# MaxLayar/Ray-Tracing-Extended

Hardware: AMD Instinct MI355X
Metric: Mrays/s (higher is better)
Workload: dtype f32; 1 GPU; configs[2]: Chess pieces x17 (100,440 triangles, BVH4), 1920x1080, 64 rays/pixel/frame (1024 spp = 16 frames), 8 bounces, PCG, FLAT_CHUNKS semantics; decomposition=single GPU, rays_per_frame=243378252, triangles=100440, chunks=7448, spheres=0

## Files before the change

ray-tracing-extended_amd/csrc/rt_api.hip:

```cpp
#include <hip/hip_runtime.h>

#include <algorithm>
#include <chrono>
#include <cfloat>
#include <cmath>
#include <condition_variable>
#include <deque>
#include <mutex>
#include <cstdarg>
#include <cstdio>
#include <cstring>
#include <ctime>
#include <string>
#include <thread>
#include <vector>

#include "rt_kernels.hpp"
#include "rt_stream.hpp"
namespace rtk {
const void* stream_kernel(bool counting, bool philox, bool compact, bool triangles);
const void* cam_stream_kernel(bool philox, bool compact, bool triangles);
}
#include "rt_geom.hpp"
#include "rt_bvh_gpu.hpp"
// ... 45 lines not shown
    size_t n_tris = 0, n_chunks = 0, n_spheres = 0;
    float sphere_mag = 0.f;
    bool geom_local = false, xf_dirty = false;
    uint64_t frames_traced = 0, frames_at_world_build = ~0ull;
    std::vector<rt_triangle>       h_local_tris;
    std::vector<rt_local_chunk>    h_lchunks;
    std::vector<rt_mesh_transform> h_xf;
    std::vector<float>             mesh_radius;
    int n_meshes = 0;
    DevBuf<float> d_local_tris;
    DevBuf<uint32_t> d_tri_mesh, d_tri_chunk, d_tri_rank, d_order;
    DevBuf<rtg::MeshXf> d_xf;
    hipEvent_t evg0 = nullptr, evg1 = nullptr;
    hipEvent_t ev_switch = nullptr;

    DevBuf<float4> d_sph_geom, d_sph_mat, d_nodes, d_nodes_h, d_tri_geo, d_tri_nrm, d_chunk_mat, d_chunk_box;
    DevBuf<float>  d_raw_tris;
    DevBuf<uint32_t> d_raw_range;
    DevBuf<float4> d_frame, d_accum;
    DevBuf<uint32_t> d_display;
    DevBuf<float4> d_batch;
    DevBuf<uint32_t> d_tile_order, d_tile_cost, d_tile_hist;
    bool lpt_active = true;
    bool tile_order_valid = false, tile_order_stale = false; int tile_order_n = 0;
    size_t target_pixels = 0;
    int target_w = 0, target_h = 0, target_row0 = 0, target_rows = 0, target_row_stride = 8;
    unsigned int* d_tile_counter = nullptr;
    unsigned long long* d_counters = nullptr;

    rtbvh::Bvh bvh;
    size_t n_nodes = 0;
    rtgb::Workspace bvh_ws;
    float area_at_build = 0.f;
    float area_after_refit = 0.f;
    int opt_device_bvh = -1;
    int opt_bvh_radius = -16;
    int opt_peer_copies = 0;
    int opt_bvh_treelet_ratio = 8, opt_bvh_treelet_isolate = 1, opt_bvh_treelet_first = 1;
    int opt_bvh_treelets = 6;
    int opt_bvh_top = 0;
    int opt_rebuild_percent = 200;
    int n_cu = 0;
    int opt_kernel = -1;
    int auto_choice = -1; double auto_ms[2] = { -1.0, -1.0 };
    unsigned variants_launched = 0;
    int opt_shade_threshold = 48;
    int opt_tile_sync = 1;
    int opt_fetch_guide = 4;
    int opt_fetch_guide_philox = 1;
    int opt_tiles_per_fetch = 16;
    int opt_compact_nodes = 1;
    int opt_stream_tile = 4;
    int opt_node_min = 10;
    int opt_blocks_per_cu = 0;
    int opt_full_sort = 0;
    int opt_tile_lpt = 1;
    int opt_frame_batch = 0;
    int opt_tile_w_log2 = 3;
    int opt_bvh_reinsert = 0;
    int opt_bvh_bins = 32, opt_bvh_cost_exp = 100;
    int opt_max_leaf = 2;
    int opt_bvh_collapse = 0;
    int opt_bvh_node_cost = 130;
    int opt_stream_stack = 0;
    int opt_lds_stack = 0;
    DevBuf<uint32_t> d_gstack;
    DevBuf<uint4> d_primary; DevBuf<float4> d_focus; DevBuf<unsigned int> d_primary_counts;
    std::string primary_key;
    unsigned long long scene_version = 0;
    int opt_primary_lists = 1;
    DevBuf<float> d_park;
    std::vector<rtk::CamRecord> h_cams; DevBuf<rtk::CamRecord> d_cams;
    DevBuf<float4> d_q_rays, d_q_hits; DevBuf<uint8_t> d_q_occ;
    DevBuf<unsigned int> d_q_bound;
    DevBuf<float4> d_aov[RT_AOV_COUNT];
    size_t aov_pixels = 0;
    int aov_w = 0, aov_h = 0, aov_row0 = 0, aov_rows = 0, aov_row_stride = 8;
    rt_aov_info aov{};
    rt_stats stats{};

    std::thread q_thread; bool q_started = false;
    std::mutex q_mu; std::condition_variable q_cv, q_idle;
    struct QItem { int frame; rt_params p; };
    std::deque<QItem> q_frames; bool q_busy = false, q_stop = false;
    rt_params q_tail{};
    int q_rc = 0; std::string q_err;
    int opt_queue_depth = 64;
    int opt_queue_linger_us = 200;
};

namespace {

int fail(rt_ctx* ctx, int code, const char* fmt, ...)
{
    char buf[512];
    va_list ap; va_start(ap, fmt); vsnprintf(buf, sizeof buf, fmt, ap); va_end(ap);
    if (ctx) ctx->err = buf; else g_create_error = buf;
    return code;
}

template <class T> hipError_t upload(rt_ctx* c, DevBuf<T>& d, const std::vector<T>& v)
{
    hipError_t e = d.ensure(v.size());
    if (e == hipSuccess && !v.empty()) e = hipMemcpyAsync(d.p, v.data(), v.size() * sizeof(T), hipMemcpyHostToDevice, c->stream);
    return e;
}
// ... 475 lines not shown
    if (philox && var == Variant::Flat) return fail(c, -2, "the flat validation kernel implements the PCG stream only");
    if (philox) kernel = 1;
    if (philox && (c->target_w > 65535 || c->target_rows > 65535)) return fail(c, -7, "the Philox mode addresses at most 65535 x 65535 pixels per context");
    if (philox && (c->params.numRaysPerPixel > 65000 || c->params.maxBounceCount > 32000))
        return fail(c, -7, "the Philox mode takes at most 65000 rays per pixel per frame and 32000 bounces (sample and bounce share one signed 32-bit register)");
    const bool stream = P.stream = kernel == 1 && var != Variant::Flat && c->params.numRaysPerPixel >= 1
                                   && c->target_w <= 65535 && c->target_rows <= 65535;
    const bool tile_kernel = P.tile_kernel = !stream && var != Variant::Flat;
    F.stack_cap = tile_kernel ? tile_stack_cap(c)
                              : std::max(1, c->bvh.maxStack) + (stream ? 3 : 0);
    const bool six_waves = stream && !philox && var == Variant::Fast && c->opt_compact_nodes != 0 && c->n_nodes > 0;
    const int stream_stack = c->opt_stream_stack > 0 ? c->opt_stream_stack : (six_waves ? 24 : 30);
    const bool stream_spill = stream && F.stack_cap > stream_stack;
    if (stream_spill) F.stack_cap = stream_stack;
    F.full_sort = c->opt_full_sort;
    bool fixed_origin = camera_origin_is_fixed(c->params);
    if (cams) for (int f = 0; f < n_frames; ++f) fixed_origin = fixed_origin && camera_origin_is_fixed(cams[f]);
    F.fixed_origin = fixed_origin ? 1 : 0;
    F.out_frame = c->d_frame.p; F.accum = c->d_accum.p;
    F.tile_counter = c->d_tile_counter; F.counters = c->d_counters;

    const size_t lds = P.lds = var == Variant::Flat ? 0
                                       : (size_t)F.stack_cap * 64 * sizeof(uint32_t) * rtk::kWavesPerBlock
                                         + (stream ? (size_t)rtk::kGroupMax * sizeof(uint2) * rtk::kWavesPerBlock : 0);
    if (lds > 160 * 1024) return fail(c, -7, "BVH needs a %d-entry traversal stack: exceeds the 160 KiB LDS", F.stack_cap);
    const bool counting = var == Variant::Counting;
    const bool compact = c->opt_compact_nodes != 0;
    P.cam_table = cams != nullptr;
    const void* fn = P.fn = var == Variant::Flat ? (const void*)rtk::k_trace<false, true>
                   : stream ? (cams ? rtk::cam_stream_kernel(philox, compact, c->n_nodes > 0)
                                    : rtk::stream_kernel(counting, philox, compact, c->n_nodes > 0))
                   : c->n_nodes == 0
                            ? dispatch3(counting, false, false, [](auto C, auto, auto) { return (const void*)rtk::k_trace<decltype(C)::value, false, false, 6>; })
                            : dispatch3(counting, false, compact, [](auto C, auto, auto H) { return (const void*)rtk::k_trace<decltype(C)::value, false, decltype(H)::value>; });
    if (lds > 64 * 1024) RT_HIP(c, hipFuncSetAttribute(fn, hipFuncAttributeMaxDynamicSharedMemorySize, (int)lds));
    int per_cu = 0;
    RT_HIP(c, hipOccupancyMaxActiveBlocksPerMultiprocessor(&per_cu, fn, rtk::kBlock, lds));
    if (per_cu < 1) return fail(c, -7, "kernel does not fit a CU (LDS %zu B)", lds);
    P.ntiles = F.tiles_x * F.tiles_y;
    P.sample_lanes_log2 = !philox ? 0 : c->params.numRaysPerPixel >= 16 ? 4 : c->params.numRaysPerPixel >= 4 ? 2 : 0;
    const bool stream_sync = P.stream_sync = stream && (c->opt_tile_sync || philox);
    if (cams && !stream_sync) return fail(c, -7, "per-frame cameras: no k_cam_stream launch for this target");
    const size_t frames_in_queue = ((stream_sync && c->opt_frame_batch != 1) ? (size_t)std::max(1, std::min(n_frames, 64)) : 1) << P.sample_lanes_log2;
    const int want = (int)std::min<size_t>(((size_t)P.ntiles * frames_in_queue + rtk::kWavesPerBlock - 1) / rtk::kWavesPerBlock, (size_t)1 << 20);
    if (c->opt_blocks_per_cu > 0) per_cu = std::min(per_cu, c->opt_blocks_per_cu);
    const int grid = P.grid = std::max(1, std::min(want, per_cu * c->n_cu));
    A.shade_threshold = std::max(1, std::min(64, c->opt_shade_threshold));
    A.total_pixels = (unsigned int)P.ntiles * 64u;
    A.tile_sync = stream_sync ? 1 : 0;
    A.sample_lanes_log2 = P.sample_lanes_log2;
    A.tiles_per_fetch = std::max(1, std::min(rtk::kGroupMax, c->opt_tiles_per_fetch));
    A.guide_div = 1;
    A.node_min = std::max(1, std::min(64, c->opt_node_min));
    const unsigned int gstack_stride = (unsigned int)grid * rtk::kBlock;
    if (philox) {
        RT_HIP(c, c->d_park.ensure((size_t)grid * rtk::kWavesPerBlock * (size_t)A.tiles_per_fetch * 192));
        F.park = c->d_park.p;
    }
    if (stream_spill) {
        RT_HIP(c, c->d_gstack.ensure((size_t)(c->bvh.maxStack + 3 - F.stack_cap) * gstack_stride));
        F.gstack = c->d_gstack.p; F.gstack_stride = gstack_stride;
    }
    if (tile_kernel && c->bvh.maxStack > F.stack_cap) {
        RT_HIP(c, c->d_gstack.ensure((size_t)(c->bvh.maxStack - F.stack_cap) * gstack_stride));
        F.gstack = c->d_gstack.p; F.gstack_stride = gstack_stride;
    }
    if ((tile_kernel || stream_sync) && n_frames > 1 && c->opt_frame_batch != 1) {
        const size_t budget = (size_t)4 << 30;
        const size_t per_frame = c->target_pixels * sizeof(float4);
        int batch = (int)std::min<size_t>((size_t)n_frames, std::max<size_t>(1, budget / per_frame));
        if (c->opt_frame_batch > 1) batch = std::min(batch, c->opt_frame_batch);
        P.batch = batch = std::min(batch, 256);
        if (batch > 1) RT_HIP(c, c->d_batch.ensure((size_t)batch * c->target_pixels));
    }
    return 0;
}

int plan_tile_order(rt_ctx* c, LaunchPlan& P)
{
    const int ntiles = P.ntiles;
    const bool lpt = (P.tile_kernel || P.stream_sync) && c->opt_tile_lpt && ntiles > 1;
    c->lpt_active = lpt;
    if (!lpt) return 0;
    if (c->tile_order_n != ntiles) { c->tile_order_valid = false; c->tile_order_n = ntiles; }
    RT_HIP(c, c->d_tile_cost.ensure(ntiles)); RT_HIP(c, c->d_tile_order.ensure(ntiles));
    if (!c->tile_order_valid || c->tile_order_stale) {
        P.record_costs = true;
        RT_HIP(c, hipMemsetAsync(c->d_tile_cost.p, 0, (size_t)ntiles * sizeof(uint32_t), c->stream));
    }
    P.F.tile_order = c->tile_order_valid ? c->d_tile_order.p : nullptr;
    P.F.tile_cost = P.record_costs ? c->d_tile_cost.p : nullptr;
    return 0;
}

int ensure_primary_lists(rt_ctx* c, LaunchPlan& P)
{
    const bool eligible = P.stream && !P.cam_table && c->opt_primary_lists && c->n_nodes > 0 && P.F.fixed_origin && c->target_pixels > 0
                          && c->bvh.maxStack <= 160;
    if (!eligible) return 0;
    std::string key((const char*)&c->params, sizeof c->params);
    const unsigned long long geo[6] = { c->scene_version, (unsigned long long)c->target_row0, (unsigned long long)c->target_rows,
                                        (unsigned long long)c->target_row_stride, (unsigned long long)c->target_w, (unsigned long long)c->target_h };
    key.append((const char*)geo, sizeof geo);
    if (key != c->primary_key) {
        RT_HIP(c, c->d_primary.ensure(c->target_pixels)); RT_HIP(c, c->d_focus.ensure(c->target_pixels)); RT_HIP(c, c->d_primary_counts.ensure(4));
        RT_HIP(c, hipMemsetAsync(c->d_primary_counts.p, 0, 4 * sizeof(unsigned int), c->stream));
// ... 615 lines not shown
    if (c->geom_local && n_meshes != c->n_meshes) return fail(c, -2, "%d transforms for %d meshes", n_meshes, c->n_meshes);
    c->h_xf.assign(xf, xf + n_meshes);
    c->xf_dirty = true;
    return 0;
}

int rt_read_world_geometry(rt_ctx* c, rt_triangle* tris_out, int n_tris, rt_meshinfo* mi_out, int n_chunks)
{
    if (!c) return -1;
    RT_SETTLE(c);
    if (!c->geom_local) return fail(c, -2, "no local meshes uploaded");
    if (!c->have_params) return fail(c, -2, "rt_set_params has not been called");
    if (n_tris != (int)c->h_local_tris.size() || n_chunks != (int)c->h_lchunks.size()) return fail(c, -2, "size mismatch");
    RT_HIP(c, hipSetDevice(c->device));
    { int r = prepare_scene(c); if (r) return r; }
    if (n_tris) RT_HIP(c, hipMemcpy(tris_out, c->d_raw_tris.p, (size_t)n_tris * sizeof(rt_triangle), hipMemcpyDeviceToHost));
    std::vector<float4> box(2 * (size_t)n_chunks);
    if (n_chunks) RT_HIP(c, hipMemcpy(box.data(), c->d_chunk_box.p, box.size() * sizeof(float4), hipMemcpyDeviceToHost));
    for (int m = 0; m < n_chunks; ++m) {
        const rt_local_chunk& ch = c->h_lchunks[m];
        rt_meshinfo& mi = mi_out[m];
        mi.firstTriangleIndex = ch.firstTriangleIndex; mi.numTriangles = ch.numTriangles; mi.material = ch.material;
        mi.boundsMin[0] = box[2 * m].x; mi.boundsMin[1] = box[2 * m].y; mi.boundsMin[2] = box[2 * m].z;
        mi.boundsMax[0] = box[2 * m + 1].x; mi.boundsMax[1] = box[2 * m + 1].y; mi.boundsMax[2] = box[2 * m + 1].z;
    }
    return 0;
}

int rt_set_option(rt_ctx* c, const char* name, int value)
{
    if (!c) return -1;
    RT_SETTLE(c);
    if (!name) return fail(c, -2, "null option name");
    if (!std::strcmp(name, "kernel")) {
        if (value < -1 || value > 1) return fail(c, -2, "kernel must be -1 (auto), 0 (k_trace) or 1 (k_stream)");
        c->opt_kernel = value;
    }
    else if (!std::strcmp(name, "shade_threshold")) { if (value < 1 || value > 64) return fail(c, -2, "shade_threshold must be in [1,64]"); c->opt_shade_threshold = value; }
    else if (!std::strcmp(name, "stream_stack")) { if (value != 0 && (value < 4 || value > 128)) return fail(c, -2, "stream_stack must be 0 (automatic) or in [4,128]"); c->opt_stream_stack = value; }
    else if (!std::strcmp(name, "lds_stack")) { if (value < 0 || value > 64) return fail(c, -2, "lds_stack must be in [0,64]"); c->opt_lds_stack = value; }
    else if (!std::strcmp(name, "bvh_bins")) { if (value < 2 || value > 128) return fail(c, -2, "bvh_bins must be in [2,128]"); if (value != c->opt_bvh_bins) c->scene_dirty = true; c->opt_bvh_bins = value; }
    else if (!std::strcmp(name, "bvh_reinsert")) { if (value < 0 || value > 16) return fail(c, -2, "bvh_reinsert must be in [0,16]"); if (value != c->opt_bvh_reinsert) c->scene_dirty = true; c->opt_bvh_reinsert = value; }
    else if (!std::strcmp(name, "bvh_cost_exp")) { if (value < 10 || value > 300) return fail(c, -2, "bvh_cost_exp must be in [10,300] (percent)"); if (value != c->opt_bvh_cost_exp) c->scene_dirty = true; c->opt_bvh_cost_exp = value; }
    else if (!std::strcmp(name, "max_leaf")) { if (value < 1 || value > rtbvh::kMaxLeaf) return fail(c, -2, "max_leaf must be in [1,4]"); if (value != c->opt_max_leaf) c->scene_dirty = true; c->opt_max_leaf = value; }
    else if (!std::strcmp(name, "bvh_collapse")) { if (value < 0 || value > 2) return fail(c, -2, "bvh_collapse must be 0 (greedy), 1 (cost-driven, leaves formed by the collapse) or 2 (cost-driven over the split search's leaves)"); if (value != c->opt_bvh_collapse) c->scene_dirty = true; c->opt_bvh_collapse = value; }
    else if (!std::strcmp(name, "bvh_node_cost")) { if (value < 1 || value > 10000) return fail(c, -2, "bvh_node_cost must be in [1,10000] (percent of a triangle test)"); if (value != c->opt_bvh_node_cost) c->scene_dirty = true; c->opt_bvh_node_cost = value; }
    else if (!std::strcmp(name, "tile_w_log2")) { if (value < 0 || value > 6) return fail(c, -2, "tile_w_log2 must be in [0,6]"); c->opt_tile_w_log2 = value; }
    else if (!std::strcmp(name, "tile_lpt")) { c->opt_tile_lpt = value ? 1 : 0; c->tile_order_valid = false; }
    else if (!std::strcmp(name, "frame_batch")) { if (value < 0 || value > 1024) return fail(c, -2, "frame_batch must be in [0,1024]"); c->opt_frame_batch = value; }
    else if (!std::strcmp(name, "fetch_guide")) { if (value < 1 || value > 64) return fail(c, -2, "fetch_guide must be in [1,64]"); c->opt_fetch_guide = value; }
    else if (!std::strcmp(name, "fetch_guide_philox")) { if (value < 1 || value > 64) return fail(c, -2, "fetch_guide_philox must be in [1,64]"); c->opt_fetch_guide_philox = value; }
    else if (!std::strcmp(name, "tiles_per_fetch")) { if (value < 1 || value > 64) return fail(c, -2, "tiles_per_fetch must be in [1,64]"); c->opt_tiles_per_fetch = value; }
    else if (!std::strcmp(name, "node_min")) { if (value < 1 || value > 64) return fail(c, -2, "node_min must be in [1,64]"); c->opt_node_min = value; }
    else if (!std::strcmp(name, "tile_sync")) c->opt_tile_sync = value ? 1 : 0;
    else if (!std::strcmp(name, "compact_nodes")) c->opt_compact_nodes = value ? 1 : 0;
    else if (!std::strcmp(name, "device_bvh")) { if (value < -1 || value > 1) return fail(c, -2, "device_bvh must be -1 (automatic), 0 or 1"); if (value != c->opt_device_bvh) c->scene_dirty = true; c->opt_device_bvh = value; }
    else if (!std::strcmp(name, "bvh_radius")) { if (value == 0 || value < -rtgb::kMaxRadius || value > rtgb::kMaxRadius) return fail(c, -2, "bvh_radius must be in [1,64] (negative: the same radius in every round)"); if (value != c->opt_bvh_radius) c->scene_dirty = true; c->opt_bvh_radius = value; }
    else if (!std::strcmp(name, "peer_copies")) { if (value != 0 && value != 1) return fail(c, -2, "peer_copies must be 0 or 1"); c->opt_peer_copies = value; }
    else if (!std::strcmp(name, "bvh_treelet_ratio")) { if (value < 2 || value > 64) return fail(c, -2, "bvh_treelet_ratio must be in [2,64]"); if (value != c->opt_bvh_treelet_ratio) c->scene_dirty = true; c->opt_bvh_treelet_ratio = value; }
    else if (!std::strcmp(name, "bvh_treelet_isolate")) { if (value < 0 || value > 1) return fail(c, -2, "bvh_treelet_isolate must be 0 or 1"); if (value != c->opt_bvh_treelet_isolate) c->scene_dirty = true; c->opt_bvh_treelet_isolate = value; }
    else if (!std::strcmp(name, "bvh_treelet_first")) { if (value < 1 || value > 4096) return fail(c, -2, "bvh_treelet_first must be in [1,4096]"); if (value != c->opt_bvh_treelet_first) c->scene_dirty = true; c->opt_bvh_treelet_first = value; }
    else if (!std::strcmp(name, "bvh_treelets")) { if (value < 0 || value > 16) return fail(c, -2, "bvh_treelets must be in [0,16] (passes)"); if (value != c->opt_bvh_treelets) c->scene_dirty = true; c->opt_bvh_treelets = value; }
    else if (!std::strcmp(name, "bvh_top")) { if (value < 0 || value > (1 << 20)) return fail(c, -2, "bvh_top must be in [0,1048576] (0 = the device's clustering builds the whole tree)"); if (value != c->opt_bvh_top) c->scene_dirty = true; c->opt_bvh_top = value; }
    else if (!std::strcmp(name, "rebuild_percent")) { if (value < 0 || value > 100000) return fail(c, -2, "rebuild_percent must be in [0,100000] (0 = never rebuild)"); c->opt_rebuild_percent = value; }
    else if (!std::strcmp(name, "stream_tile")) { if (value != 0 && value != 2 && value != 4) return fail(c, -2, "stream_tile must be 0 (8x8 pixels x 1 frame), 2 (4x4 x 4 frames) or 4 (2x2 x 16 frames)"); c->opt_stream_tile = value; }
    else if (!std::strcmp(name, "full_sort")) c->opt_full_sort = value ? 1 : 0;
    else if (!std::strcmp(name, "primary_lists")) { if (value != 0 && value != 1) return fail(c, -2, "primary_lists must be 0 or 1"); c->opt_primary_lists = value; }
    else if (!std::strcmp(name, "queue_depth")) { if (value < 1 || value > 256) return fail(c, -2, "queue_depth must be in [1,256]"); c->opt_queue_depth = value; }
    else if (!std::strcmp(name, "queue_linger_us")) { if (value < 0 || value > 1000000) return fail(c, -2, "queue_linger_us must be in [0,1000000]"); c->opt_queue_linger_us = value; }
    else if (!std::strcmp(name, "blocks_per_cu")) { if (value < 0) return fail(c, -2, "blocks_per_cu must be >= 0"); c->opt_blocks_per_cu = value; }
    else return fail(c, -2, "unknown option '%s'", name);
    return 0;
}

int rt_set_rows(rt_ctx* c, int row0, int nrows)
{
    if (!c) return -1;
    RT_SETTLE(c);
    if (row0 < 0 || nrows < 0) return fail(c, -2, "bad row strip (%d,%d)", row0, nrows);
    c->row0 = row0; c->nrows = nrows; c->band_stride = 0;
    return 0;
}

int rt_set_bands(rt_ctx* c, int first_band, int band_stride)
{
    if (!c) return -1;
    RT_SETTLE(c);
    if (first_band < 0 || band_stride < 1 || first_band >= band_stride) return fail(c, -2, "bad band pattern (%d,%d)", first_band, band_stride);
    c->band_first = first_band; c->band_stride = band_stride;
    return 0;
}

int rt_render_frame(rt_ctx* c, int frame_index) { if (!c) return -1; RT_SETTLE(c); return launch_frames(c, frame_index, 1, Variant::Fast); }
int rt_render(rt_ctx* c, int first_frame, int n_frames) { if (!c) return -1; RT_SETTLE(c); return launch_frames(c, first_frame, n_frames, Variant::Fast); }
int rt_render_counting(rt_ctx* c, int first_frame, int n_frames) { if (!c) return -1; RT_SETTLE(c); return launch_frames(c, first_frame, n_frames, Variant::Counting); }
int rt_render_frame_flat(rt_ctx* c, int frame_index) { if (!c) return -1; RT_SETTLE(c); return launch_frames(c, frame_index, 1, Variant::Flat); }

int rt_render_params(rt_ctx* c, int first_frame, int n_frames, const rt_params* params)
{
    if (!c) return -1;
    RT_SETTLE(c);
    if (n_frames < 0) return fail(c, -2, "n_frames < 0");
    if (n_frames == 0) return 0;
    if (!params) return fail(c, -2, "null params");
    if (const int f = other_settings(params, n_frames)) return fail(c, -2, "rt_render_params: entry %d differs from entry 0 outside the camera fields", f);
    if (!c->have_params || !same_settings(c->params, params[0])) { const int r = rt_set_params(c, &params[0]); if (r) return r; }
// ... 551 lines not shown
```

ray-tracing-extended_amd/csrc/rt_stream.hpp:

```cpp
#pragma once
#include "rt_kernels.hpp"

namespace rtk {

struct StreamArgs {
    int shade_threshold;
    unsigned int total_pixels;
    int node_min;
    int tiles_per_fetch;
    int guide_div;
    int tile_sync;
    int n16, n4, n1;
    int sample_lanes_log2;
};

enum : uint32_t { kModeTrav = 0, kModeShade = 1, kModeDead = 2, kModeWait = 3, kModeTravStrict = 0xFFFFFFFFu };
__device__ __forceinline__ bool is_trav(uint32_t mode) { return (int)mode <= 0; }
constexpr uint32_t kNoPixel = 0xFFFFFFFFu;

struct StreamKernArgs { DeviceScene S; FrameArgs F; StreamArgs A; };
static_assert(alignof(StreamArgs) <= 8, "kernarg layout = struct layout");
static_assert(offsetof(StreamKernArgs, F) == ((sizeof(DeviceScene) + 7) & ~size_t(7))
              && offsetof(StreamKernArgs, A) == ((offsetof(StreamKernArgs, F) + sizeof(FrameArgs) + 7) & ~size_t(7)), "kernarg layout = struct layout");

struct CamRecord {
    float4 view;
    float4 m0, m1, m2;
    float4 pos;
};
struct StreamCamKernArgs { DeviceScene S; FrameArgs F; StreamArgs A; const CamRecord* cams; };
static_assert(offsetof(StreamCamKernArgs, A) == offsetof(StreamKernArgs, A)
              && offsetof(StreamCamKernArgs, cams) == ((offsetof(StreamCamKernArgs, A) + sizeof(StreamArgs) + 7) & ~size_t(7)), "kernarg layout = struct layout");

#ifndef RT_STREAM_WAVES
#define RT_STREAM_WAVES 6
#endif
#ifndef RT_STREAM_WAVES_PHILOX
#define RT_STREAM_WAVES_PHILOX 5
#endif
constexpr int stream_waves(bool count, bool philox, bool h, bool tri) { return count ? 3 : !tri ? 6 : philox ? RT_STREAM_WAVES_PHILOX : !h ? 5 : RT_STREAM_WAVES; }


template <bool COUNT, bool PHILOX = false, bool H = false, bool TRI = true>
__global__ __launch_bounds__(kBlock) __attribute__((amdgpu_waves_per_eu(stream_waves(COUNT, PHILOX, H, TRI), stream_waves(COUNT, PHILOX, H, TRI)))) void k_stream(DeviceScene S, FrameArgs F, StreamArgs A)
{
    constexpr bool CAMS = false;
#include "rt_stream_body.hpp"
}

template <bool PHILOX, bool H, bool TRI>
__global__ __launch_bounds__(kBlock) __attribute__((amdgpu_waves_per_eu(stream_waves(false, PHILOX, H, TRI), stream_waves(false, PHILOX, H, TRI)))) void k_cam_stream(DeviceScene S, FrameArgs F, StreamArgs A, const CamRecord* cams)
{
    constexpr bool COUNT = false, CAMS = true;
    (void)cams;
#include "rt_stream_body.hpp"
}

}
```

ray-tracing-extended_amd/csrc/rt_stream_body.hpp:

```cpp
    extern __shared__ uint32_t lds_stack[];
    RT_MARK("begin prologue");
    const int lane = threadIdx.x & 63, wave = threadIdx.x >> 6;
    uint32_t* stk = lds_stack + (size_t)wave * F.stack_cap * 64 + lane;
    const int cap = F.stack_cap;
    uint32_t* const gstk = F.gstack ? F.gstack + (blockIdx.x * kBlock + threadIdx.x) : nullptr;
    using lds_u32 = __attribute__((address_space(3))) uint32_t;
    const uint32_t stk0 = (uint32_t)(uintptr_t)(lds_u32*)stk;
    uint32_t top = stk0;
    auto slot = [](uint32_t a) -> lds_u32& { return *reinterpret_cast<lds_u32*>((uintptr_t)a); };
    const uint32_t capb = (uint32_t)cap << 8;
    auto pop = [&]() -> uint32_t {
        top -= 256u;
        if (gstk == nullptr) return slot(top);
        RT_RARE_PATH();
        const uint32_t depth = top - stk0;
        uint32_t v = slot(stk0 + min(depth, capb - 256u));
        asm volatile("" : "+v"(v));
        if (depth >= capb) { RT_RARE_PATH(); v = gstk[(size_t)((depth - capb) >> 8) * F.gstack_stride]; }
        return v;
    };
    typedef uint32_t u32x2 __attribute__((ext_vector_type(2)));
    using lds_u2 = __attribute__((address_space(3))) u32x2;
    lds_u2* const item_tab = reinterpret_cast<lds_u2*>((uintptr_t)__builtin_amdgcn_readfirstlane(
                                 (uint32_t)(uintptr_t)(lds_u32*)(lds_stack + (size_t)kWavesPerBlock * F.stack_cap * 64) + (uint32_t)wave * (kGroupMax * 8u)));
    Counters cnt = {};
    const float INF = __builtin_inff();
    auto park_slot = [&](const FrameArgs& F, const StreamArgs& A, unsigned int k) -> float* {
        return F.park + (((size_t)(blockIdx.x * kWavesPerBlock) + (threadIdx.x >> 6)) * (unsigned)A.tiles_per_fetch + k) * 192u;
    };

    uint32_t mode = A.tile_sync ? kModeWait : kModeShade;
    bool fresh = false;
    uint32_t pxy = kNoPixel;
    uint32_t rng = 0u;
    int sample = 0, bounce = 0;
    v3 total = rtm::mk(0.f, 0.f, 0.f), light = total, rayColour = total, o = total, d = total;
    RaySlabT<H> slab = make_slab<H>(rtm::mk(0.f, 0.f, 0.f), rtm::mk(1.f, 1.f, 1.f));
    uint32_t cur = kNone;
    Hit best; best.t = INF; best.id = kNone; best.u = 0.f; best.v = 0.f;
    bool live = false;
    unsigned long long wave_t0 = 0;
    unsigned int group_base = 0, group_len = 0;
    unsigned int next_unit = 0;
    unsigned int kidx = 0;

    auto decode = [](const FrameArgs& F, const StreamArgs& A, unsigned int item, unsigned int& tile, unsigned int& sub, unsigned int& frame0) -> int {
        const unsigned int ntiles_ = (unsigned)(F.tiles_x * F.tiles_y);
        if constexpr (PHILOX) {
            const int sgl = A.sample_lanes_log2;
            const unsigned int per_frame = ntiles_ << sgl;
            const unsigned int g = item / per_frame, r = item - g * per_frame;
            tile = r >> sgl; sub = r & ((1u << sgl) - 1u); frame0 = g;
            return sgl;
        }
        const unsigned int items1_ = (unsigned)A.n1 * ntiles_, items4_ = (unsigned)A.n4 * (ntiles_ << 2);
        int fgl = 0; unsigned int fbase = (unsigned)A.n16 * 16u + (unsigned)A.n4 * 4u;
        if (item >= items1_) { item -= items1_; fgl = 2; fbase = (unsigned)A.n16 * 16u; if (item >= items4_) { item -= items4_; fgl = 4; fbase = 0u; } }
        const unsigned int per_group = ntiles_ << fgl;
        const unsigned int g = item / per_group, r = item - g * per_group;
        tile = r >> fgl; sub = r & ((1u << fgl) - 1u); frame0 = fbase + (g << fgl);
        return fgl;
    };
    auto pixel_index = [&](const FrameArgs& F) -> uint32_t {
        const int ly = (int)(pxy >> 16);
        return (uint32_t)(F.row0 + (ly >> 3) * F.row_stride + (ly & 7)) * (uint32_t)F.p.width + (pxy & 0xFFFFu);
    };
    auto start_pixel = [&](const FrameArgs& F, const StreamArgs& A, unsigned int id) -> bool {
        const rt_params& p = F.p;
        const uint32_t W = (uint32_t)p.width;
        const unsigned int nframes_ = (unsigned)(A.n16 * 16 + A.n4 * 4 + A.n1);
        const u32x2 e = item_tab[id >> 6];
        const unsigned int pos = id & 63u;
        const int fgl = (int)(e.y >> 28);
        const unsigned int frame0 = e.y & 0x0FFFFFFFu;
        const int pxl = 6 - fgl, swl = pxl >> 1;
        const unsigned int pix = pos & ((1u << pxl) - 1u);
        const unsigned int fi = PHILOX ? frame0 : frame0 + (pos >> pxl);
        const int x = (int)((e.x & 0xFFFFu) + (pix & ((1u << swl) - 1u)));
        const int yy = (int)((e.x >> 16) + (pix >> swl));
        if (!(x < p.width && yy < F.nrows && fi < nframes_)) return false;
        pxy = (uint32_t)x | ((uint32_t)yy << 16); kidx = id | (fi << 16);
        const uint32_t pixelIndex = (uint32_t)(F.row0 + (yy >> 3) * F.row_stride + (yy & 7)) * W + (uint32_t)x;
        if constexpr (PHILOX) sample = (int)(pos >> pxl);
        else { rng = pixelIndex + (uint32_t)(F.frame + (int)fi) * 719393u; sample = 0; }
        total = rtm::mk(0.f, 0.f, 0.f);
        live = false;
        return true;
    };
    auto take_units = [&](const FrameArgs& F, const StreamArgs& A, bool want) -> bool {
        bool got = false;
        const unsigned int total_units = group_len << 6;
        for (;;) {
            const unsigned long long need = ballot_(want);
            if (need == 0ull || next_unit >= total_units) break;
            if (want) {
                const unsigned int id = next_unit + __builtin_amdgcn_mbcnt_hi((uint32_t)(need >> 32), __builtin_amdgcn_mbcnt_lo((uint32_t)need, 0u));
                if (id < total_units && start_pixel(F, A, id)) { want = false; got = true; }
// ... 40 lines not shown
                        const float cx = tx / nf, cy = ty / nf, cz = tz / nf;
                        const size_t pi = (size_t)yy * W + (uint32_t)x;
                        F.out_frame[(size_t)fi * F.frame_stride + pi] = make_float4(cx, cy, cz, 1.0f);
                        if (F.frames_in_launch <= 1) {
                            const float weight = 1.0f / (float)(F.frame + 1);
                            const float omw = 1.0f - weight;
                            const float4 prev = F.accum[pi];
                            float4 acc;
                            acc.x = rtm::saturate(prev.x * omw + cx * weight);
                            acc.y = rtm::saturate(prev.y * omw + cy * weight);
                            acc.z = rtm::saturate(prev.z * omw + cz * weight);
                            acc.w = rtm::saturate(prev.w * omw + 1.0f * weight);
                            F.accum[pi] = acc;
                        }
                    }
                }
            }
            uint32_t slot = (uint32_t)lane;
            asm volatile("" : "+v"(slot));
            if (F.tile_cost && group_len != 0 && slot < group_len) {
                const uint32_t share = (uint32_t)(((__builtin_readcyclecounter() - wave_t0) >> 6) / group_len);
                const u32x2 e = item_tab[slot];
                atomicAdd(&F.tile_cost[((e.x >> 16) >> 3) * (unsigned)F.tiles_x + ((e.x & 0xFFFFu) >> 3)], share);
            }
            unsigned int base = 0, K = 1;
            if (lane == 0) {
                const unsigned int handed = __hip_atomic_load(F.tile_counter, __ATOMIC_RELAXED, __HIP_MEMORY_SCOPE_AGENT) >> 6;
                const unsigned int rem = nitems_ > handed ? nitems_ - handed : 0u;
                K = min((unsigned)A.tiles_per_fetch, max(1u, rem / (unsigned)A.guide_div));
                base = atomicAdd(F.tile_counter, 64u * K);
            }
            base = __builtin_amdgcn_readfirstlane(base);
            K = __builtin_amdgcn_readfirstlane(K);
            group_base = base >> 6;
            if (group_base >= nitems_) break;
            group_len = min(K, nitems_ - group_base);
            wave_t0 = __builtin_readcyclecounter();
            if (slot < group_len) {
                unsigned int tile, sub, frame0;
                const int fgl = decode(F, A, group_base + slot, tile, sub, frame0);
                const int swl = (6 - fgl) >> 1;
                if (F.tile_order) tile = F.tile_order[tile];
                const unsigned int x0 = (tile % (unsigned)F.tiles_x) * 8u + ((sub & ((1u << (3 - swl)) - 1u)) << swl);
                const unsigned int y0 = (tile / (unsigned)F.tiles_x) * 8u + ((sub >> (3 - swl)) << swl);
                item_tab[slot] = u32x2{ x0 | (y0 << 16), frame0 | ((unsigned)fgl << 28) };
            }
            next_unit = 0;
            if (take_units(F, A, true)) { fresh = true; mode = kModeShade; }
            RT_REGION_END(fetch);
            continue;
        }

        const int thr = min(A.shade_threshold, (A.shade_threshold * (nTrav + nShade) + 63) >> 6);
        if (nShade >= thr || nTrav == 0) {
            __builtin_amdgcn_s_setprio(0);
            RT_REGION_BEGIN(shade);
            const StreamKernArgs& KA = fresh_kernargs<StreamKernArgs>();
            const DeviceScene& S = KA.S; const FrameArgs& F = KA.F; const StreamArgs& A = KA.A;
            const rt_params& p = F.p;
            const float* M = p.camLocalToWorld;
            const uint32_t W = (uint32_t)p.width;
            bool need_ray = false;
            bool want = false;
            bool retrace = false;
            if (mode == kModeShade) {
                need_ray = fresh;
                fresh = false;
                bool path_done = false;
                if constexpr (TRI) {
                    if (live && best.id != kNone && (best.id & kTriBit) && p.intersectMode == RT_INTERSECT_FLAT_CHUNKS) {
                        RT_REGION_BEGIN(verify);
                        const uint32_t chunk = __float_as_uint(S.tri_nrm[(size_t)(best.id & ~kTriBit) * 3].w);
                        const float4 bmn = S.chunk_box[(size_t)chunk * 2], bmx = S.chunk_box[(size_t)chunk * 2 + 1];
                        if (!ray_bounding_box(o, slab.inv, rtm::mk(bmn.x, bmn.y, bmn.z), rtm::mk(bmx.x, bmx.y, bmx.z))) { retrace = true; live = false; }
                        RT_REGION_END(verify);
                    }
                }
                if (live) {
                    if (best.id != kNone) {
                        RT_REGION_BEGIN(hit);
                        phase_tick<COUNT>(cnt, 2);
                        if (COUNT) cnt.hits++;
                        const v3 hitPoint = o + d * best.t;
                        v3 normal; const float4* mat;
                        if (best.id & kTriBit) {
                            const uint32_t ti = best.id & ~kTriBit;
                            const float4* tn = S.tri_nrm + (size_t)ti * 3;
                            const float4 n0 = tn[0], n1 = tn[1], n2 = tn[2];
                            const float w = 1.0f - best.u - best.v;
                            normal = rtm::normalize((rtm::mk(n0.x, n0.y, n0.z) * w + rtm::mk(n1.x, n1.y, n1.z) * best.u)
                                                    + rtm::mk(n2.x, n2.y, n2.z) * best.v);
                            mat = S.chunk_mat + (size_t)__float_as_uint(n0.w) * 4;
                        } else {
                            RT_REGION_BEGIN(hit_sphere);
                            const float4 s = S.sph_geom[best.id];
                            normal = rtm::normalize(hitPoint - rtm::mk(s.x, s.y, s.z));
                            mat = S.sph_mat + (size_t)best.id * 4;
                            RT_REGION_END(hit_sphere);
                        }
                        const float4 mcol = mat[0], memi = mat[1], mprm = mat[3];
                        const int flag = (int)__float_as_uint(mprm.w);
                        v3 colour = rtm::mk(mcol.x, mcol.y, mcol.z);
                        bool skip = false;
                        if (flag == 1) {
                            RT_REGION_BEGIN(hit_checker);
                            float cx = mod2(__builtin_floorf(hitPoint.x)), cz = mod2(__builtin_floorf(hitPoint.z));
                            if (!(cx == cz)) colour = rtm::mk(memi.x, memi.y, memi.z);
                            RT_REGION_END(hit_checker);
// ... 145 lines not shown
                        if (false) {
#else
                        if (F.focus != nullptr) {
#endif
                            const float4 fpt = F.focus[(size_t)ly * W + (uint32_t)px];
                            cam.focusPoint = rtm::mk(fpt.x, fpt.y, fpt.z);
                        } else {
                        RT_MARK("begin camera_focus");
                        const float uvx = ((float)px + 0.5f) / cam.W, uvy = ((float)y + 0.5f) / (float)(uint32_t)p.height;
                        const float lx = (uvx - 0.5f) * p.viewParams[0], lyv = (uvy - 0.5f) * p.viewParams[1], lz = 1.0f * p.viewParams[2];
                        cam.focusPoint = rtm::mk(((M[0] * lx + M[1] * lyv) + M[2]  * lz) + M[3]  * 1.0f,
                                                 ((M[4] * lx + M[5] * lyv) + M[6]  * lz) + M[7]  * 1.0f,
                                                 ((M[8] * lx + M[9] * lyv) + M[10] * lz) + M[11] * 1.0f);
                        RT_MARK("end camera_focus");
                        }
                        if constexpr (PHILOX) {
                            rtm::PhiloxScope R;
                            R.begin((uint32_t)y * W + (uint32_t)px, (uint32_t)F.frame + (kidx >> 16), (uint32_t)sample & 0xFFFFu, 0u);
                            camera_ray(p, cam, R, o, d, F.fixed_origin != 0);
                        } else camera_ray(p, cam, rng, o, d, F.fixed_origin != 0);
                        }
                        if constexpr (PHILOX) sample &= 0xFFFF; else bounce = 0;
                        rayColour = rtm::mk(1.f, 1.f, 1.f); light = rtm::mk(0.f, 0.f, 0.f);
                        RT_REGION_END(camera);
                    }
                    {
                        RT_REGION_BEGIN(setup);
                        if (!retrace) cnt.rays++;
                        best.t = INF; best.id = kNone;
                        const float a = rtm::dot(d, d);
                        const SphereA sa = sphere_a(a);
                        for (int i = 0; i < S.ns; ++i) {
                            RT_REGION_BEGIN(setup_spheres);
                            const float4 s = S.sph_geom[i];
                            float dst;
                            if (COUNT && !retrace) cnt.sph++;
                            if (ray_sphere(o, d, sa, rtm::mk(s.x, s.y, s.z), s.w, dst) && dst < best.t) { best.t = dst; best.id = (uint32_t)i; }
                            RT_REGION_END(setup_spheres);
                        }
                        live = true;
                        const bool traceable = ray_traceable(o, d, a);
                        if constexpr (TRI) {
                            if (S.nn > 0 && traceable) {
                                slab = make_slab<H>(o, d);
                                cur = 0; top = stk0; mode = retrace ? kModeTravStrict : kModeTrav;
                                if (F.primary != nullptr && need_ray) {
                                    RT_REGION_BEGIN(setup_list);
                                    const uint4 L = F.primary[(size_t)(pxy >> 16) * W + (pxy & 0xFFFFu)];
                                    if (L.x != 0xFFFFFFFEu) {
                                        cur = L.x;
                                        slot(top) = L.w; top = (L.w != kNone) ? top + 256u : top;
                                        slot(top) = L.z; top = (L.z != kNone) ? top + 256u : top;
                                        slot(top) = L.y; top = (L.y != kNone) ? top + 256u : top;
                                        if (L.x == kNone) mode = kModeShade;
                                    }
                                    RT_REGION_END(setup_list);
                                }
                            }
                        }
                        RT_REGION_END(setup);
                    }
                }
            }
            RT_REGION_END(shade);
        } else {
            if constexpr (TRI) {
            __builtin_amdgcn_s_setprio(1);
            RT_REGION_BEGIN(burst);
            for (;;) {
                RT_REGION_BEGIN(burstiter);
                for (;;) {
                    RT_REGION_BEGIN(nodeloop);
                    const int nAtNode = __popcll(ballot_((int)cur >= 0));
                    if (nAtNode == 0) { RT_REGION_END(nodeloop); break; }
                    if (nAtNode < A.node_min && ballot2_(is_trav(mode), (int)cur < 0) != 0) { RT_REGION_END(nodeloop); break; }
#ifdef RT_DIAG_IDLE
                    if (COUNT) {
                        if (is_trav(mode) && (int)cur < 0) cnt.phase_lanes[3]++;
                        if (mode == kModeShade) cnt.phase_lanes[4]++;
                        if (lane == 0) { cnt.phase_execs[3]++; cnt.phase_execs[4]++; }
                    }
#endif
                    if ((int)cur >= 0) {
                        RT_REGION_BEGIN(node);
                        if (COUNT) cnt.nodes++;
                        phase_tick<COUNT>(cnt, 0);
#ifdef RT_DIAG_TOP
                        if (COUNT && cur < (uint32_t)RT_DIAG_TOP) { cnt.phase_lanes[3]++; }
                        if (COUNT && cur < 4u * RT_DIAG_TOP + 1u) { cnt.phase_lanes[4]++; }
                        if (COUNT && ballot_(cur >= (uint32_t)RT_DIAG_TOP) == 0ull && (unsigned)__builtin_ctzll(ballot_(true)) == (unsigned)lane) cnt.phase_execs[3]++;
                        if (COUNT && ballot_(cur >= 4u * RT_DIAG_TOP + 1u) == 0ull && (unsigned)__builtin_ctzll(ballot_(true)) == (unsigned)lane) cnt.phase_execs[4]++;
#endif
#ifdef RT_DIAG_PRIMARY
                        if (COUNT && (PHILOX ? (sample >> 16) : bounce) == 0) { cnt.phase_lanes[3]++; if ((unsigned)__builtin_ctzll(ballot_(true)) == (unsigned)lane) cnt.phase_execs[3]++; }
#endif
                        float t0, t1, t2, t3;
                        uint32_t c0, c1, c2, c3;
                        node_step<H>(H ? S.nodes_h : S.nodes, cur, slab, best.t, F.full_sort != 0, t0, t1, t2, t3, c0, c1, c2, c3);
                        if (gstk == nullptr || ((void)RT_RARE_PATH_EXPR(), ballot_(top - stk0 + 768u > capb) == 0)) {
                            slot(top) = c3; top = (t3 < INF) ? top + 256u : top;
                            slot(top) = c2; top = (t2 < INF) ? top + 256u : top;
                            slot(top) = c1; top = (t1 < INF) ? top + 256u : top;
                        } else {
                            RT_REGION_BEGIN(node_spill);
                            auto push = [&](uint32_t c) {
                                const uint32_t depth = top - stk0;
                                if (depth < capb) slot(top) = c; else gstk[(size_t)((depth - capb) >> 8) * F.gstack_stride] = c;
                                top += 256u;
                            };
                            if (t3 < INF) push(c3);
                            if (t2 < INF) push(c2);
                            if (t1 < INF) push(c1);
                            RT_REGION_END(node_spill);
                        }
                        if (t0 < INF) cur = c0;
                        else {
                            RT_REGION_BEGIN(node_pop);
                            if (top != stk0) cur = pop();
                            else { cur = kNone; mode = kModeShade; }
                            RT_REGION_END(node_pop);
                        }
                        RT_REGION_END(node);
                    }
                    RT_REGION_END(nodeloop);
                }
                if (is_trav(mode) && (int)cur < 0) {
                    RT_REGION_BEGIN(leaf);
                    uint32_t ti = (cur & 0x7FFFFFFFu) >> 2;
                    const uint32_t last = ti + (cur & 3u);
                    if (cur != kNone)
                    for (; ti <= last; ++ti) {
                        RT_REGION_BEGIN(tri);
                        float4 g0, g1, g2;
                        load_tri(S.tri_geo, ti, g0, g1, g2);
                        float dst, u, v;
                        if (COUNT) cnt.tris++;
                        phase_tick<COUNT>(cnt, 1);
#ifdef RT_DIAG_PRIMARY
                        if (COUNT && (PHILOX ? (sample >> 16) : bounce) == 0) { cnt.phase_lanes[4]++; if ((unsigned)__builtin_ctzll(ballot_(true)) == (unsigned)lane) cnt.phase_execs[4]++; }
#endif
                        const bool hit = ray_triangle(o, d, rtm::mk(g0.x, g0.y, g0.z), rtm::mk(g0.w, g1.x, g1.y),
                                                      rtm::mk(g1.z, g1.w, g2.x), rtm::mk(g2.y, g2.z, g2.w), dst, u, v);
                        if (hit && dst <= best.t) {
                            RT_REGION_BEGIN(tri_accept);
                            bool take = dst < best.t;
                            if (!take && (best.id & kTriBit) && best.id != kNone) {
                                RT_REGION_BEGIN(tri_tie);
                                uint32_t oc = __float_as_uint(S.tri_nrm[(size_t)ti * 3 + 1].w);
                                uint32_t ob = __float_as_uint(S.tri_nrm[(size_t)(best.id & ~kTriBit) * 3 + 1].w);
                                take = oc < ob;
                                RT_REGION_END(tri_tie);
                            }
                            if (take && mode == kModeTravStrict) {
                                RT_RARE_PATH();
                                RT_REGION_BEGIN(tri_chunk);
                                uint32_t chunk = __float_as_uint(S.tri_nrm[(size_t)ti * 3].w);
                                float4 bmn = S.chunk_box[(size_t)chunk * 2], bmx = S.chunk_box[(size_t)chunk * 2 + 1];
                                take = ray_bounding_box(o, slab.inv, rtm::mk(bmn.x, bmn.y, bmn.z), rtm::mk(bmx.x, bmx.y, bmx.z));
                                RT_REGION_END(tri_chunk);
                            }
                            if (take) { best.t = dst; best.id = kTriBit | ti; best.u = u; best.v = v; }
                            RT_REGION_END(tri_accept);
                        }
                        RT_REGION_END(tri);
                    }
                    if (top != stk0) cur = pop();
                    else { cur = kNone; mode = kModeShade; }
                    RT_REGION_END(leaf);
                }
                RT_REGION_END(burstiter);
                if (ballot_(is_trav(mode)) == 0) break;
                if ((int)__popcll(ballot_(mode == kModeShade)) >= thr) break;
            }
            RT_REGION_END(burst);
            }
        }
    }
    RT_MARK("begin epilogue");
    {
        unsigned long long v[kNumCounters] = { cnt.rays, cnt.sph, cnt.nodes, cnt.tris, cnt.hits };
        for (int k = 0; k < 5; ++k) { v[5 + k] = cnt.phase_lanes[k]; v[10 + k] = cnt.phase_execs[k]; }
        for (int k = 0; k < kNumRegions; ++k) v[15 + k] = cnt.region[k];
        for (int k = 0; k < (COUNT ? kNumCounters : 1); ++k) {
            unsigned long long s = v[k];
            for (int off = 32; off > 0; off >>= 1) s += __shfl_down(s, off, 64);
            if (lane == 0) atomicAdd(&fresh_kernargs<StreamKernArgs>().F.counters[k], s);
        }
    }
    RT_MARK("end epilogue");
```

Measured before the change: 20120 Mrays/s.

## Prioritize primary-list rays with lower shade threshold and bounded early-shade rounds

Measured after the change: 20140 Mrays/s (median of 6 runs). No clear change (+0.1%).

```diff
diff --git a/ray-tracing-extended_amd/csrc/rt_api.hip b/ray-tracing-extended_amd/csrc/rt_api.hip
--- a/ray-tracing-extended_amd/csrc/rt_api.hip
+++ b/ray-tracing-extended_amd/csrc/rt_api.hip
@@ -121,6 +121,8 @@
     int opt_compact_nodes = 1;
     int opt_stream_tile = 4;
     int opt_node_min = 10;
+    int opt_shade_rounds = 1;
+    int opt_list_shade_min = 8;
     int opt_blocks_per_cu = 0;
     int opt_full_sort = 0;
     int opt_tile_lpt = 1;
@@ -702,6 +704,8 @@
     A.tiles_per_fetch = std::max(1, std::min(rtk::kGroupMax, c->opt_tiles_per_fetch));
     A.guide_div = 1;
     A.node_min = std::max(1, std::min(64, c->opt_node_min));
+    A.shade_rounds = std::max(0, std::min(rtk::kMaxShadeRounds, c->opt_shade_rounds));
+    A.list_shade_min = std::max(1, std::min(64, c->opt_list_shade_min));
     const unsigned int gstack_stride = (unsigned int)grid * rtk::kBlock;
     if (philox) {
         RT_HIP(c, c->d_park.ensure((size_t)grid * rtk::kWavesPerBlock * (size_t)A.tiles_per_fetch * 192));
@@ -1423,6 +1427,8 @@
     else if (!std::strcmp(name, "fetch_guide_philox")) { if (value < 1 || value > 64) return fail(c, -2, "fetch_guide_philox must be in [1,64]"); c->opt_fetch_guide_philox = value; }
     else if (!std::strcmp(name, "tiles_per_fetch")) { if (value < 1 || value > 64) return fail(c, -2, "tiles_per_fetch must be in [1,64]"); c->opt_tiles_per_fetch = value; }
     else if (!std::strcmp(name, "node_min")) { if (value < 1 || value > 64) return fail(c, -2, "node_min must be in [1,64]"); c->opt_node_min = value; }
+    else if (!std::strcmp(name, "shade_rounds")) { if (value < 0 || value > rtk::kMaxShadeRounds) return fail(c, -2, "shade_rounds must be in [0,8]"); c->opt_shade_rounds = value; }
+    else if (!std::strcmp(name, "list_shade_min")) { if (value < 1 || value > 64) return fail(c, -2, "list_shade_min must be in [1,64]"); c->opt_list_shade_min = value; }
     else if (!std::strcmp(name, "tile_sync")) c->opt_tile_sync = value ? 1 : 0;
     else if (!std::strcmp(name, "compact_nodes")) c->opt_compact_nodes = value ? 1 : 0;
     else if (!std::strcmp(name, "device_bvh")) { if (value < -1 || value > 1) return fail(c, -2, "device_bvh must be -1 (automatic), 0 or 1"); if (value != c->opt_device_bvh) c->scene_dirty = true; c->opt_device_bvh = value; }
diff --git a/ray-tracing-extended_amd/csrc/rt_stream.hpp b/ray-tracing-extended_amd/csrc/rt_stream.hpp
--- a/ray-tracing-extended_amd/csrc/rt_stream.hpp
+++ b/ray-tracing-extended_amd/csrc/rt_stream.hpp
@@ -12,11 +12,14 @@
     int tile_sync;
     int n16, n4, n1;
     int sample_lanes_log2;
+    int shade_rounds;
+    int list_shade_min;
 };
 
-enum : uint32_t { kModeTrav = 0, kModeShade = 1, kModeDead = 2, kModeWait = 3, kModeTravStrict = 0xFFFFFFFFu };
+enum : uint32_t { kModeTrav = 0, kModeShade = 1, kModeDead = 2, kModeWait = 3, kModeTravStrict = 0xFFFFFFFFu, kModeTravList = 0xFFFFFFFEu };
 __device__ __forceinline__ bool is_trav(uint32_t mode) { return (int)mode <= 0; }
 constexpr uint32_t kNoPixel = 0xFFFFFFFFu;
+constexpr int kMaxShadeRounds = 8;
 
 struct StreamKernArgs { DeviceScene S; FrameArgs F; StreamArgs A; };
 static_assert(alignof(StreamArgs) <= 8, "kernarg layout = struct layout");
diff --git a/ray-tracing-extended_amd/csrc/rt_stream_body.hpp b/ray-tracing-extended_amd/csrc/rt_stream_body.hpp
--- a/ray-tracing-extended_amd/csrc/rt_stream_body.hpp
+++ b/ray-tracing-extended_amd/csrc/rt_stream_body.hpp
@@ -43,6 +43,7 @@
     unsigned int group_base = 0, group_len = 0;
     unsigned int next_unit = 0;
     unsigned int kidx = 0;
+    int list_rounds = 0;
 
     auto decode = [](const FrameArgs& F, const StreamArgs& A, unsigned int item, unsigned int& tile, unsigned int& sub, unsigned int& frame0) -> int {
         const unsigned int ntiles_ = (unsigned)(F.tiles_x * F.tiles_y);
@@ -189,8 +190,9 @@
         }
 
         const int thr = min(A.shade_threshold, (A.shade_threshold * (nTrav + nShade) + 63) >> 6);
-        if (nShade >= thr || nTrav == 0) {
+        if (nShade >= thr || nTrav == 0 || list_rounds >= 256) {
             __builtin_amdgcn_s_setprio(0);
+            list_rounds &= 255;
             RT_REGION_BEGIN(shade);
             const StreamKernArgs& KA = fresh_kernargs<StreamKernArgs>();
             const DeviceScene& S = KA.S; const FrameArgs& F = KA.F; const StreamArgs& A = KA.A;
@@ -442,7 +444,7 @@
                                         slot(top) = L.w; top = (L.w != kNone) ? top + 256u : top;
                                         slot(top) = L.z; top = (L.z != kNone) ? top + 256u : top;
                                         slot(top) = L.y; top = (L.y != kNone) ? top + 256u : top;
-                                        if (L.x == kNone) mode = kModeShade;
+                                        mode = (L.x == kNone) ? kModeShade : kModeTravList;
                                     }
                                     RT_REGION_END(setup_list);
                                 }
@@ -457,13 +459,15 @@
             if constexpr (TRI) {
             __builtin_amdgcn_s_setprio(1);
             RT_REGION_BEGIN(burst);
+            bool list_first = F.primary != nullptr && list_rounds < A.shade_rounds && ballot2_(mode == kModeTravList, (int)cur < 0) != 0ull;
             for (;;) {
                 RT_REGION_BEGIN(burstiter);
+                const int node_min = list_first ? 65 : A.node_min;
                 for (;;) {
                     RT_REGION_BEGIN(nodeloop);
                     const int nAtNode = __popcll(ballot_((int)cur >= 0));
                     if (nAtNode == 0) { RT_REGION_END(nodeloop); break; }
-                    if (nAtNode < A.node_min && ballot2_(is_trav(mode), (int)cur < 0) != 0) { RT_REGION_END(nodeloop); break; }
+                    if (nAtNode < node_min && ballot2_(is_trav(mode), (int)cur < 0) != 0) { RT_REGION_END(nodeloop); break; }
 #ifdef RT_DIAG_IDLE
                     if (COUNT) {
                         if (is_trav(mode) && (int)cur < 0) cnt.phase_lanes[3]++;
@@ -559,8 +563,14 @@
                     RT_REGION_END(leaf);
                 }
                 RT_REGION_END(burstiter);
-                if (ballot_(is_trav(mode)) == 0) break;
-                if ((int)__popcll(ballot_(mode == kModeShade)) >= thr) break;
+                const int nDone = (int)__popcll(ballot_(mode == kModeShade));
+                bool stop = ballot_(is_trav(mode)) == 0ull || nDone >= thr;
+                if (list_first) {
+                    list_first = ballot2_(mode == kModeTravList, (int)cur < 0) != 0ull;
+                    stop = !list_first && nDone >= min(thr, A.list_shade_min);
+                    if (stop) list_rounds += 257;
+                } else if (stop) list_rounds = 0;
+                if (stop) break;
             }
             RT_REGION_END(burst);
             }
```
